# HengWeiBin/CenterFusionDetect3D

Hardware: AMD Instinct MI355X
Metric: frames/sec/GPU CenterFusion forward, 3x448x800 bs=16; 1/2/4/8-GPU scaling (higher is better)
Workload: dtype f32 storage + f32 accumulate; products as split-operand MFMA passes: f16x3 backbone/neck (3 passes), heads' first 3x3 layers fp16 main term + block-scaled FP6 e2m3 cross terms (1.5 passes), heads' 1x1 layers bf16x3; 1 GPU; Centerfusion_Middle (DLA-34 + DCNv2 neck + pc_dep frustum fusion, 7+4 heads) forward + NMS/top-100 decode + 2D->3D postProcess, bs=16/GPU, 3x448x800, 50-200 radar pts/frame, random-init weights; global_batch=16, parallelism=dp1 (batch shard, async all-gather of the final boxes)

## Files before the change

centerfusiondetect3d_amd/csrc/cf_heads.hip:

```cpp
#include <string>
#include "cf_common.h"
#include "cf_mx.h"

namespace {

typedef __bf16 bf16x8 __attribute__((ext_vector_type(8)));
typedef unsigned int u32x4 __attribute__((ext_vector_type(4)));
typedef unsigned int u32x2 __attribute__((ext_vector_type(2)));
typedef _Float16 hf16x8 __attribute__((ext_vector_type(8)));
typedef int i32x8 __attribute__((ext_vector_type(8)));

constexpr int HT_PX = 64;
constexpr int HT_C = 256;
constexpr int HT_ROWB = HT_C * 2 + 16;
constexpr int HT_PLANE = HT_PX * HT_ROWB;
constexpr int HT_LDS = 2 * HT_PLANE;

struct HeadTailK {
  const unsigned char* x;
  int x_stride;
  int M, HW;
  int n_heads;
  int n_hidden;
  const unsigned char* w_hidden[CF_MAX_HEADS][2];
// ... 36 lines not shown
        hi[e] = bf16_rne(v[e]);
      }
      unsigned char* o = xt + (ct * 16 + c16) * HT_ROWB + ch * 2;
      const u32x2 ph = {pack2(hi[0], hi[1]), pack2(hi[2], hi[3])};
      const u32x2 pl = {pack2(v[0] - hi[0], v[1] - hi[1]), pack2(v[2] - hi[2], v[3] - hi[3])};
      *reinterpret_cast<u32x2*>(o) = ph;
      *reinterpret_cast<u32x2*>(o + HT_PLANE) = pl;
    }
  }
}

struct TileMap {
  int b, y0, x0, H, W, sh = 4;
  __device__ __forceinline__ bool operator()(int px, int& bb, int& pix) const {
    const int y = y0 + (px >> sh), x = x0 + (px & ((1 << sh) - 1));
    if (y >= H || x >= W) return false;
    bb = b;
    pix = y * W + x;
    return true;
  }
};

constexpr int AT_SLOTS = CF_HEAD_AT_SLOTS;
__device__ __forceinline__ int at_slot_of(int ty, int tx) { return (ty % 3 == 0 && tx % 3 == 0) ? (ty / 3) * 6 + tx / 3 : -1; }
struct SlotMap {
  const int* slots;
  int M, HW, half;
  __device__ __forceinline__ bool operator()(int px, int& bb, int& pix) const {
    const int t = half * 64 + px, sl = at_slot_of(t >> 4, t & 15);
    if (sl < 0) return false;
    const int s = slots[sl];
    if ((unsigned)s >= (unsigned)M) return false;
    bb = s / HW;
    pix = s - bb * HW;
    return true;
  }
};

template <class PixMap, int CTS = 0xF>
__device__ __forceinline__ void head_tail_from_lds16(const HeadTailK& p, unsigned char* xt, int head, const PixMap& pm) {
  const int tid = threadIdx.x, lane = tid & 63, wave = tid >> 6;
  const int g = lane >> 4, c16 = lane & 15;
  for (int l = 0; l < p.n_hidden; ++l) {
    const unsigned char* w = p.w_hidden[head][l];
    const float* bias = p.b_hidden[head][l];
    f32x4 acc[4][4];
#pragma unroll
    for (int a = 0; a < 4; ++a)
#pragma unroll
      for (int b = 0; b < 4; ++b)
#pragma unroll
        for (int r = 0; r < 4; ++r) acc[a][b][r] = 0.0f;
    bf16x8 wh[2][4], wl[2][4];
#pragma unroll
    for (int rt = 0; rt < 4; ++rt) {
      wh[0][rt] = *wfrag(w, wave * 4 + rt, 0, 0, 8, lane);
      wl[0][rt] = *wfrag(w, wave * 4 + rt, 0, 1, 8, lane);
    }
#pragma unroll
    for (int ks = 0; ks < 8; ++ks) {
      if (ks + 1 < 8) {
#pragma unroll
        for (int rt = 0; rt < 4; ++rt) {
          wh[(ks + 1) & 1][rt] = *wfrag(w, wave * 4 + rt, ks + 1, 0, 8, lane);
          wl[(ks + 1) & 1][rt] = *wfrag(w, wave * 4 + rt, ks + 1, 1, 8, lane);
        }
      }
      bf16x8 xh[4], xl[4];
#pragma unroll
      for (int ct = 0; ct < 4; ++ct) {
        if (!((CTS >> ct) & 1)) continue;
        const unsigned char* row = xt + (ct * 16 + c16) * HT_ROWB + (ks * 32 + g * 8) * 2;
        xh[ct] = *reinterpret_cast<const bf16x8*>(row);
        xl[ct] = *reinterpret_cast<const bf16x8*>(row + HT_PLANE);
      }
#pragma unroll
      for (int rt = 0; rt < 4; ++rt)
#pragma unroll
        for (int ct = 0; ct < 4; ++ct)
          if ((CTS >> ct) & 1) acc[rt][ct] = __builtin_amdgcn_mfma_f32_16x16x32_bf16(wl[ks & 1][rt], xh[ct], acc[rt][ct], 0, 0, 0);
#pragma unroll
      for (int rt = 0; rt < 4; ++rt)
#pragma unroll
        for (int ct = 0; ct < 4; ++ct)
          if ((CTS >> ct) & 1) acc[rt][ct] = __builtin_amdgcn_mfma_f32_16x16x32_bf16(wh[ks & 1][rt], xl[ct], acc[rt][ct], 0, 0, 0);
#pragma unroll
      for (int rt = 0; rt < 4; ++rt)
#pragma unroll
        for (int ct = 0; ct < 4; ++ct)
          if ((CTS >> ct) & 1) acc[rt][ct] = __builtin_amdgcn_mfma_f32_16x16x32_bf16(wh[ks & 1][rt], xh[ct], acc[rt][ct], 0, 0, 0);
      __builtin_amdgcn_sched_barrier(0);
    }
    __syncthreads();
    store_hidden_tile16<false, CTS>(xt, acc, bias, wave, lane);
    __syncthreads();
  }

  f32x4 oacc[4];
#pragma unroll
  for (int b = 0; b < 4; ++b)
#pragma unroll
    for (int r = 0; r < 4; ++r) oacc[b][r] = 0.0f;
  {
    const unsigned char* w = p.w_out[head];
#pragma unroll
    for (int s2 = 0; s2 < 2; ++s2) {
      const int ks = wave * 2 + s2;
      const bf16x8 ah = *wfrag(w, 0, ks, 0, 8, lane), al = *wfrag(w, 0, ks, 1, 8, lane);
#pragma unroll
      for (int ct = 0; ct < 4; ++ct) {
        if (!((CTS >> ct) & 1)) continue;
        const unsigned char* row = xt + (ct * 16 + c16) * HT_ROWB + (ks * 32 + g * 8) * 2;
        const bf16x8 xh = *reinterpret_cast<const bf16x8*>(row);
// ... 25 lines not shown
      const float raw = red[n * HT_PX + px] + red[(16 + n) * HT_PX + px] + red[(32 + n) * HT_PX + px] +
                        red[(48 + n) * HT_PX + px] + bo[n];
      const size_t o = ((size_t)b * n_out + n) * p.HW + pix;
      float v = raw;
      if (act == CF_ACT_RELU) v = fmaxf(raw, 0.0f);
      else if (act == CF_ACT_SIGMOID_CLAMP) v = fminf(fmaxf(cf_sigmoid(raw), 1e-4f), 1.0f - 1e-4f);
      out[o] = v;
      if (act == CF_ACT_RAW_AND_SIGDEPTH) out2[o] = 1.0f / (cf_sigmoid(raw) + 1e-6f) - 1.0f;
    }
  }
}

constexpr int HP_ROWS = (8 + 2) * (16 + 2);
constexpr int HP_PX = 8 * 16;
constexpr int HP16_RED = 4 * 16 * HP_PX * 4;
constexpr int hp16_patch_bytes(bool pc) { return HP_ROWS * (4 * 64 + (pc ? 32 : 0) + 16); }
constexpr int HP_PCIMG_ROWB = 32 * 2 + 16;
constexpr int HP_PCIMG = HP_PX * 2 * HP_PCIMG_ROWB;
constexpr int hp16_pc_extra(bool pc) { return pc ? 16 + HP_PCIMG : 0; }
constexpr int hp16_lds(bool pc, bool hidden) {
  return hidden ? (HT_LDS > hp16_patch_bytes(pc) + hp16_pc_extra(pc) ? HT_LDS : hp16_patch_bytes(pc) + hp16_pc_extra(pc))
                : hp16_patch_bytes(pc) + hp16_pc_extra(pc) + HP16_RED;
}

struct HeadPatchK {
  HeadTailK t;
  const unsigned char* src[2];
  int src_c[2];
  int H, W, tiles_x, tiles_y, n_ks;
  int pc_skip;
  int hloop;
  const unsigned char* w_first[CF_MAX_HEADS];
  const float* b_first[CF_MAX_HEADS];
  const unsigned char* w_out_perm[CF_MAX_HEADS];
  float first_scale[CF_MAX_HEADS];
  const int* slot_pixels;
};

template <int NS, bool PC, bool TP, bool MX = false, int HID = -1, bool AT = false>
__global__ __launch_bounds__(256, 2) void head_patch16_kernel(HeadPatchK q) {
  static_assert(NS == 4, "64 feature channels");
  static_assert(!AT || !TP, "virtual tiles are laid out on the flat 8 x 16 tile");
  constexpr int MX_SLAB = 14592, PC_OFF = MX ? 272 : NS * 64;
  constexpr int TSH = TP ? 3 : 4, TMASK = (1 << TSH) - 1;
  constexpr int T_H = TP ? 16 : 8, T_W = TP ? 8 : 16, P_W = T_W + 2;
  static_assert((T_H + 2) * P_W == HP_ROWS, "both tile shapes have the same patch size");
  constexpr int ROWB = NS * 64 + (PC ? 32 : 0) + 16;
  constexpr int NKF = 9 * NS / 2;
  constexpr int NK = NKF + (PC ? 1 : 0);
  extern __shared__ __attribute__((aligned(16))) unsigned char xt[];
  const HeadTailK& p = q.t;
  const int tid = threadIdx.x, lane = tid & 63, wave = __builtin_amdgcn_readfirstlane(tid >> 6);
  const int g = lane >> 4;
  const int c16 = (MX && !TP) ? ((lane & 12) == 4 || (lane & 12) == 8 ? (((lane & 15) - 4) & 3) * 4 + (((lane & 15) - 4) >> 2)
                                                                      : (lane & 3) * 4 + 2 + ((lane & 15) >> 3))
                              : (lane & 15);
  const int per_img = q.tiles_x * q.tiles_y;
  const int per_head = AT ? per_img : per_img * (p.M / p.HW);
  const int hg = blockIdx.x / per_head;
  int rem = cf_xcd_remap(blockIdx.x - hg * per_head, per_head);
  const int head0 = hg * q.hloop, head1 = min(head0 + q.hloop, p.n_heads);
  const int b = rem / per_img;
  rem -= b * per_img;
  const int y0 = (rem / q.tiles_x) * T_H, x0 = (rem % q.tiles_x) * T_W;
  const int* const at_slots = AT ? q.slot_pixels + (size_t)rem * AT_SLOTS : nullptr;
  constexpr auto live = [](int ct) { return !AT || ct % 3 == 0; };
  auto at_src = [&](int row) -> int {
    const int pr = row / P_W, pc = row % P_W;
    if (pr >= 9) return -1;
    const int s = at_slots[(pr / 3) * 6 + pc / 3];
    if ((unsigned)s >= (unsigned)p.M) return -1;
    const int bb = s / p.HW, pix = s - bb * p.HW;
    const int y = pix / q.W + pr % 3 - 1, x = pix % q.W + pc % 3 - 1;
    if ((unsigned)y >= (unsigned)q.H || (unsigned)x >= (unsigned)q.W) return -1;
    return bb * p.HW + y * q.W + x;
  };
  if constexpr (AT) {
    int any = 0;
    for (int i = 0; i < AT_SLOTS; ++i) any |= (unsigned)at_slots[i] < (unsigned)p.M ? 1 : 0;
    if (!any) return;
  }

  if constexpr (MX) {
    constexpr int UPR = 17;
    constexpr int NIT = (HP_ROWS * UPR + 255) / 256;
    u32x4 v[NIT];
#pragma unroll
    for (int it = 0; it < NIT; ++it) {
      const int idx = tid + it * 256;
      const int row = idx / UPR, u = idx % UPR;
      const int y = y0 - 1 + row / P_W, x = x0 - 1 + row % P_W;
      v[it] = u32x4{0u, 0u, 0u, 0u};
      if constexpr (AT) {
        const int s = row < HP_ROWS ? at_src(row) : -1;
        if (s >= 0) v[it] = *reinterpret_cast<const u32x4*>(q.src[0] + (size_t)s * 272 + u * 16);
      } else
      if (row < HP_ROWS && (unsigned)y < (unsigned)q.H && (unsigned)x < (unsigned)q.W)
        v[it] = *reinterpret_cast<const u32x4*>(q.src[0] + (size_t)(b * p.HW + y * q.W + x) * 272 + u * 16);
    }
#pragma unroll
    for (int it = 0; it < NIT; ++it) {
      const int idx = tid + it * 256;
      const int row = idx / UPR, u = idx % UPR;
      if (row < HP_ROWS) *reinterpret_cast<u32x4*>(xt + row * ROWB + u * 16) = v[it];
    }
  } else {
    constexpr int UPR = NS * 4;
    constexpr int NIT = (HP_ROWS * UPR + 255) / 256;
    u32x4 v[NIT];
#pragma unroll
    for (int it = 0; it < NIT; ++it) {
      const int idx = tid + it * 256;
      const int row = idx / UPR, u = idx % UPR;
      const int y = y0 - 1 + row / P_W, x = x0 - 1 + row % P_W;
      v[it] = u32x4{0u, 0u, 0u, 0u};
      if constexpr (AT) {
        const int s = row < HP_ROWS ? at_src(row) : -1;
        if (s >= 0) v[it] = *reinterpret_cast<const u32x4*>(q.src[0] + ((size_t)s * 2 * q.src_c[0]) * 2 +
                                                             (u / (NS * 2)) * q.src_c[0] * 2 + (u % (NS * 2)) * 16);
      } else
      if (row < HP_ROWS && (unsigned)y < (unsigned)q.H && (unsigned)x < (unsigned)q.W)
        v[it] = *reinterpret_cast<const u32x4*>(q.src[0] + ((size_t)(b * p.HW + y * q.W + x) * 2 * q.src_c[0]) * 2 +
                                                (u / (NS * 2)) * q.src_c[0] * 2 + (u % (NS * 2)) * 16);
    }
#pragma unroll
    for (int it = 0; it < NIT; ++it) {
      const int idx = tid + it * 256;
      const int row = idx / UPR, u = idx % UPR;
      const int plane = u / (NS * 2), uu = u % (NS * 2);
      if (row < HP_ROWS) *reinterpret_cast<u32x4*>(xt + row * ROWB + (uu >> 1) * 64 + plane * 32 + (uu & 1) * 16) = v[it];
    }
  }
  unsigned* const pc_flags = reinterpret_cast<unsigned*>(xt + hp16_patch_bytes(PC));
  if (PC) {
    unsigned nz = 0u;
    for (int idx = tid; idx < HP_ROWS * 2; idx += 256) {
      const int row = idx >> 1, plane = idx & 1;
      const int y = y0 - 1 + row / P_W, x = x0 - 1 + row % P_W;
      u32x4 w = {0u, 0u, 0u, 0u};
      if constexpr (AT) {
        const int s = at_src(row);
        if (s >= 0) w = *reinterpret_cast<const u32x4*>(q.src[1] + ((size_t)s * 2 + plane) * q.src_c[1] * 2);
      } else
      if ((unsigned)y < (unsigned)q.H && (unsigned)x < (unsigned)q.W)
        w = *reinterpret_cast<const u32x4*>(q.src[1] + ((size_t)(b * p.HW + y * q.W + x) * 2 + plane) * q.src_c[1] * 2);
      *reinterpret_cast<u32x4*>(xt + row * ROWB + PC_OFF + plane * 16) = w;
      nz |= (w[0] | w[1] | w[2] | w[3]) & 0x7fff7fffu;
    }
    const bool wave_nz = __builtin_amdgcn_ballot_w64(nz != 0u) != 0ull;
    if (lane == 0) pc_flags[wave] = (wave_nz || !q.pc_skip) ? 1u : 0u;
  }

  int rowb[8];
#pragma unroll
  for (int ct = 0; ct < 8; ++ct)
    rowb[ct] = ((c16 >> TSH) * P_W + (c16 & TMASK)) * ROWB + ct * ((16 >> TSH) * P_W * ROWB);
  const int koff = (g >> 1) * 64 + (g & 1) * 16;
  unsigned char* const pcimg = xt + hp16_patch_bytes(PC) + 16;
  const int imgb = c16 * (2 * HP_PCIMG_ROWB) + g * 16;
  __syncthreads();
  bool pc_live = false;
  if (PC) {
    const u32x4 f = *reinterpret_cast<const u32x4*>(pc_flags);
    pc_live = __builtin_amdgcn_readfirstlane((int)(f[0] | f[1] | f[2] | f[3])) != 0;
  }
  if (PC && pc_live) {
    const int ipx = tid & (HP_PX - 1), plane = tid >> 7;
    const unsigned char* sp = xt + ((ipx >> TSH) * P_W + (ipx & TMASK)) * ROWB + PC_OFF + plane * 16;
    unsigned e[32];
#pragma unroll
    for (int t = 0; t < 9; ++t) {
      const u32x2 w = *reinterpret_cast<const u32x2*>(sp + ((t / 3) * P_W + t % 3) * ROWB);
      e[3 * t] = w[0] & 0xffffu;
      e[3 * t + 1] = w[0] >> 16;
      e[3 * t + 2] = w[1] & 0xffffu;
    }
#pragma unroll
    for (int k = 27; k < 32; ++k) e[k] = 0u;
    unsigned char* dp = pcimg + (ipx * 2 + plane) * HP_PCIMG_ROWB;
#pragma unroll
    for (int j = 0; j < 4; ++j)
      *reinterpret_cast<u32x4*>(dp + j * 16) = u32x4{e[8 * j] | (e[8 * j + 1] << 16), e[8 * j + 2] | (e[8 * j + 3] << 16),
                                                     e[8 * j + 4] | (e[8 * j + 5] << 16), e[8 * j + 6] | (e[8 * j + 7] << 16)};
    __syncthreads();
  }
  auto pc_kstep = [&](const bf16x8 (&ah)[4], const bf16x8 (&al)[4], f32x4 (&acc)[4][8]) __attribute__((always_inline)) {
#pragma unroll
    for (int hf = 0; hf < 2; ++hf) {
      bf16x8 xh[4], xl[4];
#pragma unroll
      for (int ct = 0; ct < 4; ++ct) {
        if (!live(4 * hf + ct)) continue;
        const unsigned char* r = pcimg + imgb + (4 * hf + ct) * (16 * 2 * HP_PCIMG_ROWB);
        xh[ct] = *reinterpret_cast<const bf16x8*>(r);
        xl[ct] = *reinterpret_cast<const bf16x8*>(r + HP_PCIMG_ROWB);
      }
#pragma unroll
      for (int rt = 0; rt < 4; ++rt)
#pragma unroll
        for (int ct = 0; ct < 4; ++ct)
          if (live(4 * hf + ct))
            acc[rt][4 * hf + ct] = __builtin_amdgcn_mfma_f32_16x16x32_bf16(al[rt], xh[ct], acc[rt][4 * hf + ct], 0, 0, 0);
#pragma unroll
      for (int rt = 0; rt < 4; ++rt)
#pragma unroll
        for (int ct = 0; ct < 4; ++ct)
// ... 160 lines not shown
        for (int ct = 0; ct < 4; ++ct)
          if (live(4 * hf + ct))
            acc[rt][4 * hf + ct] = __builtin_amdgcn_mfma_f32_16x16x32_bf16(wh[ks & 1][rt], xl[ct], acc[rt][4 * hf + ct], 0, 0, 0);
#pragma unroll
      for (int rt = 0; rt < 4; ++rt)
#pragma unroll
        for (int ct = 0; ct < 4; ++ct)
          if (live(4 * hf + ct))
            acc[rt][4 * hf + ct] = __builtin_amdgcn_mfma_f32_16x16x32_bf16(wh[ks & 1][rt], xh[ct], acc[rt][4 * hf + ct], 0, 0, 0);
    }
    __builtin_amdgcn_sched_barrier(0);
  }
  if (PC) {
    if (pc_live) pc_kstep(wh[NKF & 1], wl[NKF & 1], acc);
  }
  };

  if (HID < 0 ? p.n_hidden > 0 : HID == 1) {
    const int head = head0;
    f32x4 acc[4][8];
    first_layer(head, acc);
    __syncthreads();
#pragma unroll
    for (int half = 0; half < 2; ++half) {
      f32x4 a2[4][4];
#pragma unroll
      for (int rt = 0; rt < 4; ++rt)
#pragma unroll
        for (int ct = 0; ct < 4; ++ct) a2[rt][ct] = acc[rt][4 * half + ct];
      if constexpr (AT) {
        if (half == 0) store_hidden_tile16<MX, 0x9>(xt, a2, q.b_first[head], wave, lane, MX ? q.first_scale[head] : 1.0f, c16);
        else store_hidden_tile16<MX, 0x4>(xt, a2, q.b_first[head], wave, lane, MX ? q.first_scale[head] : 1.0f, c16);
      } else
      store_hidden_tile16<MX>(xt, a2, q.b_first[head], wave, lane, MX ? q.first_scale[head] : 1.0f, c16);
      if constexpr (MX) __builtin_amdgcn_sched_barrier(0);
      __syncthreads();
      if constexpr (AT) {
        if (half == 0) head_tail_from_lds16<SlotMap, 0x9>(p, xt, head, SlotMap{at_slots, p.M, p.HW, half});
        else head_tail_from_lds16<SlotMap, 0x4>(p, xt, head, SlotMap{at_slots, p.M, p.HW, half});
      }
      else head_tail_from_lds16(p, xt, head, TileMap{b, y0 + (64 >> TSH) * half, x0, q.H, q.W, TSH});
      __syncthreads();
    }
    return;
  }
  if constexpr (HID == 1) return;

  for (int head = head0; head < head1; ++head) {
  f32x4 acc[4][8];
  first_layer(head, acc);
  f32x4 oacc[8];
#pragma unroll
  for (int c = 0; c < 8; ++c)
#pragma unroll
    for (int r = 0; r < 4; ++r) oacc[c][r] = 0.0f;
  {
    const float* b1 = q.b_first[head] + wave * 64 + 4 * g;
    const unsigned char* wo = q.w_out_perm[head];
    const float fsc = MX ? q.first_scale[head] : 1.0f;
    (void)fsc;
#pragma unroll
    for (int s2 = 0; s2 < 2; ++s2) {
      const int ks2 = wave * 2 + s2;
      const bf16x8 ah = *wfrag(wo, 0, ks2, 0, 8, lane), al = *wfrag(wo, 0, ks2, 1, 8, lane);
      const f32x4 ba = *reinterpret_cast<const f32x4*>(b1 + 32 * s2);
      const f32x4 bb = *reinterpret_cast<const f32x4*>(b1 + 32 * s2 + 16);
#pragma unroll
      for (int ct = 0; ct < 8; ++ct) {
        if (!live(ct)) continue;
        float v[8], hi[8];
#pragma unroll
        for (int j = 0; j < 8; ++j) {
          const float bj = j < 4 ? ba[j] : bb[j - 4];
          v[j] = fmaxf(MX ? __builtin_fmaf(acc[2 * s2 + (j >> 2)][ct][j & 3], fsc, bj) : acc[2 * s2 + (j >> 2)][ct][j & 3] + bj, 0.0f);
          hi[j] = bf16_rne(v[j]);
        }
        const u32x4 ph = {pack2(hi[0], hi[1]), pack2(hi[2], hi[3]), pack2(hi[4], hi[5]), pack2(hi[6], hi[7])};
        const u32x4 pl = {pack2(v[0] - hi[0], v[1] - hi[1]), pack2(v[2] - hi[2], v[3] - hi[3]),
                          pack2(v[4] - hi[4], v[5] - hi[5]), pack2(v[6] - hi[6], v[7] - hi[7])};
        const bf16x8 xh = __builtin_bit_cast(bf16x8, ph), xl = __builtin_bit_cast(bf16x8, pl);
        oacc[ct] = __builtin_amdgcn_mfma_f32_16x16x32_bf16(al, xh, oacc[ct], 0, 0, 0);
        oacc[ct] = __builtin_amdgcn_mfma_f32_16x16x32_bf16(ah, xl, oacc[ct], 0, 0, 0);
        oacc[ct] = __builtin_amdgcn_mfma_f32_16x16x32_bf16(ah, xh, oacc[ct], 0, 0, 0);
      }
    }
  }
  const int n_out = p.n_out[head], act = p.act[head];
  float* red = reinterpret_cast<float*>(xt + hp16_patch_bytes(PC) + hp16_pc_extra(PC));
#pragma unroll
  for (int ct = 0; ct < 8; ++ct)
#pragma unroll
    for (int r = 0; r < 4; ++r) {
      const int n = 4 * g + r;
      if (live(ct) && n < n_out) red[(wave * 16 + n) * HP_PX + ct * 16 + c16] = oacc[ct][r];
    }
  __syncthreads();
  {
    const int px = tid & (HP_PX - 1);
    const int y = y0 + (px >> TSH), x = x0 + (px & TMASK);
    bool valid = y < q.H && x < q.W;
    int ob = b;
    size_t opix = (size_t)y * q.W + x;
    if constexpr (AT) {
      const int sl = at_slot_of(px >> 4, px & 15);
      const int s = sl >= 0 ? at_slots[sl] : -1;
      valid = (unsigned)s < (unsigned)p.M;
      ob = s / p.HW;
      opix = (size_t)(s - ob * p.HW);
    }
    if (valid) {
      const float* bo = p.b_out[head];
      float* out = p.out[head];
      float* out2 = p.out2[head];
      for (int n = tid >> 7; n < n_out; n += 2) {
        const float raw = red[n * HP_PX + px] + red[(16 + n) * HP_PX + px] + red[(32 + n) * HP_PX + px] +
                          red[(48 + n) * HP_PX + px] + bo[n];
        const size_t o = ((size_t)ob * n_out + n) * p.HW + opix;
        float v = raw;
        if (act == CF_ACT_RELU) v = fmaxf(raw, 0.0f);
        else if (act == CF_ACT_SIGMOID_CLAMP) v = fminf(fmaxf(cf_sigmoid(raw), 1e-4f), 1.0f - 1e-4f);
        out[o] = v;
        if (act == CF_ACT_RAW_AND_SIGDEPTH) out2[o] = 1.0f / (cf_sigmoid(raw) + 1e-6f) - 1.0f;
      }
    }
  }
  __syncthreads();
  }
}

__global__ __launch_bounds__(256) void pack_feat_mx_kernel(const float* __restrict__ x, int in_stride,
                                                           unsigned char* __restrict__ rows, long M, float scale) {
  const long t = (long)blockIdx.x * 256 + threadIdx.x;
  const long m = t >> 1;
  const int blk = (int)(t & 1);
  if (m >= M) return;
  const f32x4* src = reinterpret_cast<const f32x4*>(x + m * in_stride + 32 * blk);
  float v[32];
#pragma unroll
  for (int i = 0; i < 8; ++i) {
// ... 96 lines not shown
  CF_REQUIRE(mx || a->K_pad / 16 >= (a->n_src == 2 ? 38 : 36), "cf_head_fused: K_pad=%d too small for the 3x3 layout", a->K_pad);
  for (int i = 0; i < n_heads; ++i) {
    CF_REQUIRE(!mx || (a->first_scale[i] > 0.0f && a->first_scale[i] < 1e30f), "cf_head_fused: head %d: first_scale missing (mx)", i);
    hp.first_scale[i] = a->first_scale[i];
  }
  if (m16) {
    CF_REQUIRE(mx || (a->K_pad % 32 == 0 && a->K_pad / 32 >= (a->n_src == 2 ? 19 : 18)), "cf_head_fused: K_pad=%d (16x16x32 fragments)", a->K_pad);
    for (int i = 0; i < n_heads; ++i)
      CF_REQUIRE(a->tail.n_out[i] <= 16, "cf_head_fused: head %d: n_out=%d > 16 (the 16x16x32 kernels produce ONE 16-row output tile, with or without hidden layers)", i, a->tail.n_out[i]);
  }
  for (int i = 0; i < n_heads; ++i) {
    CF_REQUIRE(a->tail.n_hidden > 0 || a->w_out_perm[i], "cf_head_fused: head %d: w_out_perm missing", i);
    hp.w_out_perm[i] = reinterpret_cast<const unsigned char*>(a->w_out_perm[i]);
  }
  const long t_land = (long)((W + 15) / 16) * ((H + 7) / 8), t_port = (long)((W + 7) / 8) * ((H + 15) / 16);
  CF_REQUIRE(t_land * a->tail.B * n_heads < (1L << 31), "cf_head_fused: grid too large");
  CF_REQUIRE(m16, CF_HEAD_FORMS ": nothing reads 32x32x16 fragments (mfma16 = 0)");
  bool portrait = tile < 0 ? t_port < t_land : tile != 0;
  if (at) portrait = false;
  hp.pc_skip = pc_skip != 0;
  hp.tiles_x = portrait ? (W + 7) / 8 : (W + 15) / 16;
  hp.tiles_y = portrait ? (H + 15) / 16 : (H + 7) / 8;
  const int n_img = at ? 1 : a->tail.B;
  if (at) { hp.tiles_x = n_tiles; hp.tiles_y = 1; }
  int hloop = 1;
  if (a->tail.n_hidden == 0) {
    static const int slots = [] {
      int dev = 0, cus = 256;
      if (hipGetDevice(&dev) == hipSuccess) (void)hipDeviceGetAttribute(&cus, hipDeviceAttributeMultiprocessorCount, dev);
      return 2 * (cus > 0 ? cus : 256);
    }();
    const long tiles = (long)hp.tiles_x * hp.tiles_y * n_img;
    const int n = n_heads, cand[3] = {1, 2, (n + 1) / 2};
    double best = 0.0;
    for (int i = 0; i < 3; ++i) {
      const int h = cand[i] < 1 ? 1 : (cand[i] > n ? n : cand[i]);
      const double cost = (double)((tiles * ((n + h - 1) / h) + slots - 1) / slots) * (h + 0.25);
      if (i == 0 || cost < best - 1e-9) { best = cost; hloop = h; }
    }
  }
  hp.hloop = hloop;
  const long blocks = (long)hp.tiles_x * hp.tiles_y * n_img * ((n_heads + hloop - 1) / hloop);
  CF_REQUIRE(blocks < (1L << 31), "%s: grid too large", at ? "cf_head_fused_at" : "cf_head_fused");
  const bool hidden = a->tail.n_hidden > 0;
  const bool pc = a->n_src == 2;
  const int lds = hp16_lds(pc, hidden);
  auto launch = [&](auto kernel, CfLdsLimit& lim) {
    lim.ensure(kernel, lds, hp16_lds(pc, false));
    hipLaunchKernelGGL(kernel, dim3((unsigned)blocks), dim3(256), lds, (hipStream_t)stream, hp);
  };
  static CfLdsLimit lim16[4], limx[4], limxh[2], lim_at[4];
  if (at) {
    CF_REQUIRE(!mx || hidden == pc, "cf_head_fused_at: mx = 1 runs without hidden layers and pc_hm source, or with both (the forms "
                                    "the model's head groups take); pack other heads for bf16x3");
    if (mx && hidden) launch(head_patch16_kernel<4, true, false, true, 1, true>, lim_at[3]);
    else if (mx) launch(head_patch16_kernel<4, false, false, true, 0, true>, lim_at[2]);
    else if (pc) launch(head_patch16_kernel<4, true, false, false, -1, true>, lim_at[1]);
    else launch(head_patch16_kernel<4, false, false, false, -1, true>, lim_at[0]);
    return cf_check_launch("cf_head_fused_at");
  }
  if (mx && hidden) {
    CF_REQUIRE(pc, "cf_head_fused: mx = 1 with hidden layers needs the pc_hm source (n_src = 2); pack such heads for bf16x3");
    if (portrait) launch(head_patch16_kernel<4, true, true, true, 1>, limxh[1]);
    else launch(head_patch16_kernel<4, true, false, true, 1>, limxh[0]);
  } else if (mx) {
    if (pc && portrait) launch(head_patch16_kernel<4, true, true, true, 0>, limx[3]);
    else if (pc) launch(head_patch16_kernel<4, true, false, true, 0>, limx[2]);
    else if (portrait) launch(head_patch16_kernel<4, false, true, true, 0>, limx[1]);
    else launch(head_patch16_kernel<4, false, false, true, 0>, limx[0]);
  } else {
    if (pc && portrait) launch(head_patch16_kernel<4, true, true>, lim16[3]);
    else if (pc) launch(head_patch16_kernel<4, true, false>, lim16[2]);
    else if (portrait) launch(head_patch16_kernel<4, false, true>, lim16[1]);
    else launch(head_patch16_kernel<4, false, false>, lim16[0]);
  }
  return cf_check_launch("cf_head_fused");
}

// ... 54 lines not shown
```

centerfusiondetect3d_amd/plan.py:

```python
import ctypes as C
import weakref
from typing import Dict, List

import torch

from . import _lib, ops, packing
from .pending import PendingOutputs
from ._lib import (ACT_NONE, ACT_RELU, ACT_SIGMOID_CLAMP, ACT_RAW_AND_SIGDEPTH, LAYOUT_NHWC, LAYOUT_NCHW)
from .streams import _side_streams

SECONDARY_HEADS = ["velocity", "nuscenes_att", "depth2", "rotation2"]
AT_SLOTS = 18
AT_TIMED = ("at.topk", "at.peaks", "at.tables", "at.primary")


def feat_operand(model):
    if not model._heads_bf():
        return None
    return ((packing.MX_ROW,), torch.uint8) if model._mx_active else ((2, 64), torch.bfloat16)


def act_of(h):
    return ACT_SIGMOID_CLAMP if h == "heatmap" else (ACT_RAW_AND_SIGDEPTH if h in ("depth", "depth2") else ACT_NONE)

# ... 580 lines not shown
                    self.steps[self.frustum_step] = (lib.cf_frustum_assoc, self.tk_inds.data_ptr(), K, *geom)
            self._radar_outputs(y, out, heads, pc_dep, pc_hm)
        for name, (flops, px_flops, _) in self.group_flops.items():
            self.step_flops[name] = flops
        if at is None:
            self._launch(st)
        else:
            raw = tk[:3] if self.frustum else (None, None, None)
            fused = (hm.data_ptr(), B, heads["heatmap"], h4, w4, K, *raw, pk_s.data_ptr(), pk_i.data_ptr(), pk_c.data_ptr(),
                     at["tab_ab"].data_ptr() if self.frustum else None, at["tab_b"].data_ptr(), at["ws"].data_ptr())
            self._launch(st, self._at_seq(at, (_peaks_fused_and_checksum, lib, fused, peaks[3])))
            y = self._pending(y, model, written)
        if self.peaks_step is not None and peaks_on:
            hm._cf_peaks = (K, hm.data_ptr(), pk_s, pk_i, pk_c, pk_sum)
            if self._side is not None:
                for t in (hm, pk_s, pk_i, pk_c, pk_sum):
                    t.record_stream(self._side)
        return [y]

    def _at_seq(self, at, peaks):
        lib, idx = self.lib, self.step_index
        tab_b, n_b = at["tab_b"].data_ptr(), at["n_b"]
        tab_p, n_p = (at["tab_ab"].data_ptr(), at["n_ab"]) if self.frustum else (tab_b, n_b)
        HP_PX = 48
        extra = ([("at.topk", (_no_launch,), 0)] if self.frustum else []) + [
                  ("at.peaks", peaks, 0), ("at.tables", (_no_launch,), 0),
                  ("at.primary", (lib.cf_head_fused_at, C.byref(at["f_rest"]), tab_p, n_p), 0)]
        repl = {idx["tails.primary"]: (lib.cf_head_fused, C.byref(at["f_hm"]))}
        self.step_flops["tails.primary"] = at["flops_hm"]
        self.step_flops["at.primary"] = n_p * HP_PX * at["px_rest"]
        for name in ("tails.chained", "tails.secondary"):
            if name in idx:
                _, px_flops, f = self.group_flops[name]
                repl[idx[name]] = (lib.cf_head_fused_at, C.byref(f), tab_b, n_b)
                self.step_flops[name] = n_b * HP_PX * px_flops
        seq = []
        for i, (step, lane) in enumerate(zip(self.steps, self.lanes)):
            seq.append((i, repl.get(i, step), lane))
            if i == idx["tails.primary"]:
                seq += extra
        return seq

    def _pending(self, y, model, written):
        fwd = torch.cuda.current_stream(self.device)
        lib, dev = self.lib, self.device
        names = [n for n in ("tails.primary", "tails.chained", "tails.secondary") if n in self.step_index]
        blocks = []
        for n in names:
            f = self.group_flops[n][2]
            c = _lib.HeadFusedArgs()
            C.memmove(C.byref(c), C.byref(f), C.sizeof(f))
            blocks.append(c)
        bufs = {t.data_ptr(): t for n in names for t in self.group_srcs[n]}
        keep = [written, list(y.values()), self, model._packed, bufs]

        def materialise():
            with torch.cuda.device(dev):
                for c in blocks:
# ... 48 lines not shown
```

Baseline: 3180 frames/s.

## Pack listed AT pixels densely into 48-pixel workgroups with paired-head blocks

The attention-tail head kernels stop mapping listed pixels onto a sparse 8x16 virtual tile (one live pixel per 3x3 cell). They now pack 48 listed pixels contiguously per workgroup, each with its own 9-row neighbourhood patch. A small LDS table holds each pixel's flat index and packed y/x. The hidden chain deepens its weight prefetch to three k-steps, and a 512-thread paired-head variant runs two heads at once when the grid oversubscribes the CUs. This cuts wasted MFMA columns, gather work and block count for the sparse decode-time head evaluation, at the cost of more LDS per block, new occupancy heuristics and extra register pressure from the deeper prefetch.

```diff
diff --git a/centerfusiondetect3d_amd/csrc/cf_heads.hip b/centerfusiondetect3d_amd/csrc/cf_heads.hip
--- a/centerfusiondetect3d_amd/csrc/cf_heads.hip
+++ b/centerfusiondetect3d_amd/csrc/cf_heads.hip
@@ -82,22 +82,25 @@
 };
 
 constexpr int AT_SLOTS = CF_HEAD_AT_SLOTS;
-__device__ __forceinline__ int at_slot_of(int ty, int tx) { return (ty % 3 == 0 && tx % 3 == 0) ? (ty / 3) * 6 + tx / 3 : -1; }
+constexpr int AT_S = 48;
+constexpr int AT_CTS = (1 << (AT_S / 16)) - 1;
+constexpr int AT_AHEAD = 3;
+constexpr int AT_ROWS = 9 * AT_S;
+constexpr int AT_INFO = AT_S * 8;
 struct SlotMap {
-  const int* slots;
-  int M, HW, half;
+  const int* info;
+  int HW;
   __device__ __forceinline__ bool operator()(int px, int& bb, int& pix) const {
-    const int t = half * 64 + px, sl = at_slot_of(t >> 4, t & 15);
-    if (sl < 0) return false;
-    const int s = slots[sl];
-    if ((unsigned)s >= (unsigned)M) return false;
+    if (px >= AT_S) return false;
+    const int s = info[2 * px];
+    if (s < 0) return false;
     bb = s / HW;
     pix = s - bb * HW;
     return true;
   }
 };
 
-template <class PixMap, int CTS = 0xF>
+template <class PixMap, int CTS = 0xF, int AHEAD = 1>
 __device__ __forceinline__ void head_tail_from_lds16(const HeadTailK& p, unsigned char* xt, int head, const PixMap& pm) {
   const int tid = threadIdx.x, lane = tid & 63, wave = tid >> 6;
   const int g = lane >> 4, c16 = lane & 15;
@@ -111,19 +114,22 @@
       for (int b = 0; b < 4; ++b)
 #pragma unroll
         for (int r = 0; r < 4; ++r) acc[a][b][r] = 0.0f;
-    bf16x8 wh[2][4], wl[2][4];
-#pragma unroll
-    for (int rt = 0; rt < 4; ++rt) {
-      wh[0][rt] = *wfrag(w, wave * 4 + rt, 0, 0, 8, lane);
-      wl[0][rt] = *wfrag(w, wave * 4 + rt, 0, 1, 8, lane);
-    }
+    constexpr int NB = AHEAD + 1;
+    bf16x8 wh[NB][4], wl[NB][4];
+#pragma unroll
+    for (int a = 0; a < AHEAD; ++a)
+#pragma unroll
+      for (int rt = 0; rt < 4; ++rt) {
+        wh[a][rt] = *wfrag(w, wave * 4 + rt, a, 0, 8, lane);
+        wl[a][rt] = *wfrag(w, wave * 4 + rt, a, 1, 8, lane);
+      }
 #pragma unroll
     for (int ks = 0; ks < 8; ++ks) {
-      if (ks + 1 < 8) {
+      if (ks + AHEAD < 8) {
 #pragma unroll
         for (int rt = 0; rt < 4; ++rt) {
-          wh[(ks + 1) & 1][rt] = *wfrag(w, wave * 4 + rt, ks + 1, 0, 8, lane);
-          wl[(ks + 1) & 1][rt] = *wfrag(w, wave * 4 + rt, ks + 1, 1, 8, lane);
+          wh[(ks + AHEAD) % NB][rt] = *wfrag(w, wave * 4 + rt, ks + AHEAD, 0, 8, lane);
+          wl[(ks + AHEAD) % NB][rt] = *wfrag(w, wave * 4 + rt, ks + AHEAD, 1, 8, lane);
         }
       }
       bf16x8 xh[4], xl[4];
@@ -138,17 +144,17 @@
       for (int rt = 0; rt < 4; ++rt)
 #pragma unroll
         for (int ct = 0; ct < 4; ++ct)
-          if ((CTS >> ct) & 1) acc[rt][ct] = __builtin_amdgcn_mfma_f32_16x16x32_bf16(wl[ks & 1][rt], xh[ct], acc[rt][ct], 0, 0, 0);
+          if ((CTS >> ct) & 1) acc[rt][ct] = __builtin_amdgcn_mfma_f32_16x16x32_bf16(wl[ks % NB][rt], xh[ct], acc[rt][ct], 0, 0, 0);
 #pragma unroll
       for (int rt = 0; rt < 4; ++rt)
 #pragma unroll
         for (int ct = 0; ct < 4; ++ct)
-          if ((CTS >> ct) & 1) acc[rt][ct] = __builtin_amdgcn_mfma_f32_16x16x32_bf16(wh[ks & 1][rt], xl[ct], acc[rt][ct], 0, 0, 0);
+          if ((CTS >> ct) & 1) acc[rt][ct] = __builtin_amdgcn_mfma_f32_16x16x32_bf16(wh[ks % NB][rt], xl[ct], acc[rt][ct], 0, 0, 0);
 #pragma unroll
       for (int rt = 0; rt < 4; ++rt)
 #pragma unroll
         for (int ct = 0; ct < 4; ++ct)
-          if ((CTS >> ct) & 1) acc[rt][ct] = __builtin_amdgcn_mfma_f32_16x16x32_bf16(wh[ks & 1][rt], xh[ct], acc[rt][ct], 0, 0, 0);
+          if ((CTS >> ct) & 1) acc[rt][ct] = __builtin_amdgcn_mfma_f32_16x16x32_bf16(wh[ks % NB][rt], xh[ct], acc[rt][ct], 0, 0, 0);
       __builtin_amdgcn_sched_barrier(0);
     }
     __syncthreads();
@@ -220,6 +226,16 @@
   return hidden ? (HT_LDS > hp16_patch_bytes(pc) + hp16_pc_extra(pc) ? HT_LDS : hp16_patch_bytes(pc) + hp16_pc_extra(pc))
                 : hp16_patch_bytes(pc) + hp16_pc_extra(pc) + HP16_RED;
 }
+constexpr int at_patch_bytes(bool pc) { return AT_ROWS * (4 * 64 + (pc ? 32 : 0) + 16); }
+constexpr int at_pc_extra(bool pc) { return pc ? 16 + AT_S * 2 * HP_PCIMG_ROWB : 0; }
+constexpr int AT_RED = 4 * 16 * AT_S * 4;
+constexpr int at_lds(bool pc, bool hidden, bool pair = false) {
+  return at_patch_bytes(pc) + at_pc_extra(pc) + AT_INFO + (hidden ? 0 : (pair ? 2 : 1) * AT_RED);
+}
+constexpr int CU_LDS = 160 * 1024;
+static_assert(at_lds(true, false) <= CU_LDS && at_lds(true, true) <= CU_LDS && at_lds(false, false, true) <= CU_LDS,
+              "an AT workgroup's patch, operand image and partial sums fit one CU's LDS");
+static_assert(at_patch_bytes(false) >= HT_LDS, "the hidden chain's tile lies inside the AT patch");
 
 struct HeadPatchK {
   HeadTailK t;
@@ -233,22 +249,30 @@
   const unsigned char* w_out_perm[CF_MAX_HEADS];
   float first_scale[CF_MAX_HEADS];
   const int* slot_pixels;
+  int n_slots;
 };
 
-template <int NS, bool PC, bool TP, bool MX = false, int HID = -1, bool AT = false>
-__global__ __launch_bounds__(256, 2) void head_patch16_kernel(HeadPatchK q) {
+template <int NS, bool PC, bool TP, bool MX = false, int HID = -1, bool AT = false, bool PAIR = false>
+__global__ __launch_bounds__(PAIR ? 512 : 256, PAIR ? 1 : 2) void head_patch16_kernel(HeadPatchK q) {
+  static_assert(!PAIR || (AT && MX && !PC && HID == 0), "paired heads: the mx listed-pixel form without hidden layers");
+  constexpr int NT = PAIR ? 512 : 256;
   static_assert(NS == 4, "64 feature channels");
-  static_assert(!AT || !TP, "virtual tiles are laid out on the flat 8 x 16 tile");
+  static_assert(!AT || !TP, "listed pixels have no tile orientation");
   constexpr int MX_SLAB = 14592, PC_OFF = MX ? 272 : NS * 64;
   constexpr int TSH = TP ? 3 : 4, TMASK = (1 << TSH) - 1;
-  constexpr int T_H = TP ? 16 : 8, T_W = TP ? 8 : 16, P_W = T_W + 2;
-  static_assert((T_H + 2) * P_W == HP_ROWS, "both tile shapes have the same patch size");
+  constexpr int T_H = TP ? 16 : 8, T_W = TP ? 8 : 16, P_W = AT ? 3 : T_W + 2;
+  static_assert(AT || (T_H + 2) * P_W == HP_ROWS, "both tile shapes have the same patch size");
   constexpr int ROWB = NS * 64 + (PC ? 32 : 0) + 16;
+  constexpr int NROWS = AT ? AT_ROWS : HP_ROWS, NPX = AT ? AT_S : HP_PX;
+  constexpr int PATCH = NROWS * ROWB, INFO_OFF = PATCH + (PC ? 16 + NPX * 2 * HP_PCIMG_ROWB : 0), RED_OFF = INFO_OFF + (AT ? AT_INFO : 0);
+  static_assert(AT ? PATCH == at_patch_bytes(PC) && INFO_OFF == PATCH + at_pc_extra(PC)
+                   : PATCH == hp16_patch_bytes(PC) && RED_OFF == PATCH + hp16_pc_extra(PC), "the launcher's LDS figures");
   constexpr int NKF = 9 * NS / 2;
   constexpr int NK = NKF + (PC ? 1 : 0);
   extern __shared__ __attribute__((aligned(16))) unsigned char xt[];
   const HeadTailK& p = q.t;
-  const int tid = threadIdx.x, lane = tid & 63, wave = __builtin_amdgcn_readfirstlane(tid >> 6);
+  const int tid = threadIdx.x, lane = tid & 63, wave = PAIR ? __builtin_amdgcn_readfirstlane(tid >> 6) & 3 : __builtin_amdgcn_readfirstlane(tid >> 6);
+  const int grp = PAIR ? __builtin_amdgcn_readfirstlane(tid >> 8) : 0;
   const int g = lane >> 4;
   const int c16 = (MX && !TP) ? ((lane & 12) == 4 || (lane & 12) == 8 ? (((lane & 15) - 4) & 3) * 4 + (((lane & 15) - 4) >> 2)
                                                                       : (lane & 3) * 4 + 2 + ((lane & 15) >> 3))
@@ -261,25 +285,62 @@
   const int b = rem / per_img;
   rem -= b * per_img;
   const int y0 = (rem / q.tiles_x) * T_H, x0 = (rem % q.tiles_x) * T_W;
-  const int* const at_slots = AT ? q.slot_pixels + (size_t)rem * AT_SLOTS : nullptr;
-  constexpr auto live = [](int ct) { return !AT || ct % 3 == 0; };
+  const int at_first = AT ? rem * AT_S : 0;
+  int* const at_info = reinterpret_cast<int*>(xt + INFO_OFF);
+  constexpr auto live = [](int ct) { return !AT || ct < AT_S / 16; };
   auto at_src = [&](int row) -> int {
-    const int pr = row / P_W, pc = row % P_W;
-    if (pr >= 9) return -1;
-    const int s = at_slots[(pr / 3) * 6 + pc / 3];
-    if ((unsigned)s >= (unsigned)p.M) return -1;
-    const int bb = s / p.HW, pix = s - bb * p.HW;
-    const int y = pix / q.W + pr % 3 - 1, x = pix % q.W + pc % 3 - 1;
-    if ((unsigned)y >= (unsigned)q.H || (unsigned)x >= (unsigned)q.W) return -1;
-    return bb * p.HW + y * q.W + x;
+    const int sl = row / 9, t = row - sl * 9;
+    const u32x2 inf = *reinterpret_cast<const u32x2*>(at_info + 2 * sl);
+    const int dy = t / 3 - 1, dx = t % 3 - 1;
+    const int y = (int)(inf[1] >> 16) + dy, x = (int)(inf[1] & 0xffffu) + dx;
+    if ((int)inf[0] < 0 || (unsigned)y >= (unsigned)q.H || (unsigned)x >= (unsigned)q.W) return -1;
+    return (int)inf[0] + dy * q.W + dx;
   };
   if constexpr (AT) {
-    int any = 0;
-    for (int i = 0; i < AT_SLOTS; ++i) any |= (unsigned)at_slots[i] < (unsigned)p.M ? 1 : 0;
-    if (!any) return;
-  }
-
-  if constexpr (MX) {
+    if (tid < AT_S) {
+      const int s = at_first + tid < q.n_slots ? q.slot_pixels[at_first + tid] : -1;
+      int flat = -1, yx = 0;
+      if ((unsigned)s < (unsigned)p.M) {
+        const int pix = s % p.HW, y = pix / q.W;
+        flat = s;
+        yx = (y << 16) | (pix - y * q.W);
+      }
+      at_info[2 * tid] = flat;
+      at_info[2 * tid + 1] = yx;
+    }
+    __syncthreads();
+    static_assert(AT_S <= 64, "one lane per entry");
+    if (__builtin_amdgcn_ballot_w64(lane < AT_S && at_info[2 * (lane < AT_S ? lane : 0)] >= 0) == 0ull) return;
+  }
+
+  if constexpr (AT) {
+    constexpr int UPR = MX ? 17 : NS * 4;
+    constexpr int NU = AT_ROWS * UPR, NIT = (NU + NT - 1) / NT, BATCH = 8;
+#pragma unroll
+    for (int b0 = 0; b0 < NIT; b0 += BATCH) {
+      u32x4 v[BATCH];
+#pragma unroll
+      for (int j = 0; j < BATCH; ++j) {
+        if (b0 + j >= NIT) continue;
+        const int idx = min(tid + (b0 + j) * NT, NU - 1);
+        const int row = idx / UPR, u = idx % UPR;
+        const int s = at_src(row), sc = max(s, 0);
+        v[j] = MX ? *reinterpret_cast<const u32x4*>(q.src[0] + (size_t)sc * 272 + u * 16)
+                  : *reinterpret_cast<const u32x4*>(q.src[0] + ((size_t)sc * 2 * q.src_c[0]) * 2 +
+                                                    (u / (NS * 2)) * q.src_c[0] * 2 + (u % (NS * 2)) * 16);
+        if (s < 0) v[j] = u32x4{0u, 0u, 0u, 0u};
+      }
+#pragma unroll
+      for (int j = 0; j < BATCH; ++j) {
+        const int idx = tid + (b0 + j) * NT;
+        const int row = idx / UPR, u = idx % UPR;
+        const int plane = u / (NS * 2), uu = u % (NS * 2);
+        if (b0 + j < NIT && idx < NU)
+          *reinterpret_cast<u32x4*>(xt + row * ROWB + (MX ? u * 16 : (uu >> 1) * 64 + plane * 32 + (uu & 1) * 16)) = v[j];
+      }
+      __builtin_amdgcn_sched_barrier(0);
+    }
+  } else if constexpr (MX) {
     constexpr int UPR = 17;
     constexpr int NIT = (HP_ROWS * UPR + 255) / 256;
     u32x4 v[NIT];
@@ -289,10 +350,6 @@
       const int row = idx / UPR, u = idx % UPR;
       const int y = y0 - 1 + row / P_W, x = x0 - 1 + row % P_W;
       v[it] = u32x4{0u, 0u, 0u, 0u};
-      if constexpr (AT) {
-        const int s = row < HP_ROWS ? at_src(row) : -1;
-        if (s >= 0) v[it] = *reinterpret_cast<const u32x4*>(q.src[0] + (size_t)s * 272 + u * 16);
-      } else
       if (row < HP_ROWS && (unsigned)y < (unsigned)q.H && (unsigned)x < (unsigned)q.W)
         v[it] = *reinterpret_cast<const u32x4*>(q.src[0] + (size_t)(b * p.HW + y * q.W + x) * 272 + u * 16);
     }
@@ -312,11 +369,6 @@
       const int row = idx / UPR, u = idx % UPR;
       const int y = y0 - 1 + row / P_W, x = x0 - 1 + row % P_W;
       v[it] = u32x4{0u, 0u, 0u, 0u};
-      if constexpr (AT) {
-        const int s = row < HP_ROWS ? at_src(row) : -1;
-        if (s >= 0) v[it] = *reinterpret_cast<const u32x4*>(q.src[0] + ((size_t)s * 2 * q.src_c[0]) * 2 +
-                                                             (u / (NS * 2)) * q.src_c[0] * 2 + (u % (NS * 2)) * 16);
-      } else
       if (row < HP_ROWS && (unsigned)y < (unsigned)q.H && (unsigned)x < (unsigned)q.W)
         v[it] = *reinterpret_cast<const u32x4*>(q.src[0] + ((size_t)(b * p.HW + y * q.W + x) * 2 * q.src_c[0]) * 2 +
                                                 (u / (NS * 2)) * q.src_c[0] * 2 + (u % (NS * 2)) * 16);
@@ -329,17 +381,30 @@
       if (row < HP_ROWS) *reinterpret_cast<u32x4*>(xt + row * ROWB + (uu >> 1) * 64 + plane * 32 + (uu & 1) * 16) = v[it];
     }
   }
-  unsigned* const pc_flags = reinterpret_cast<unsigned*>(xt + hp16_patch_bytes(PC));
+  unsigned* const pc_flags = reinterpret_cast<unsigned*>(xt + PATCH);
   if (PC) {
     unsigned nz = 0u;
-    for (int idx = tid; idx < HP_ROWS * 2; idx += 256) {
+    if constexpr (AT) {
+      constexpr int NITP = (NROWS * 2 + 255) / 256;
+      u32x4 w[NITP];
+#pragma unroll
+      for (int it = 0; it < NITP; ++it) {
+        const int idx = min(tid + it * 256, NROWS * 2 - 1);
+        const int s = at_src(idx >> 1);
+        w[it] = *reinterpret_cast<const u32x4*>(q.src[1] + ((size_t)max(s, 0) * 2 + (idx & 1)) * q.src_c[1] * 2);
+        if (s < 0 || tid + it * 256 >= NROWS * 2) w[it] = u32x4{0u, 0u, 0u, 0u};
+      }
+#pragma unroll
+      for (int it = 0; it < NITP; ++it) {
+        const int idx = tid + it * 256;
+        if (idx < NROWS * 2) *reinterpret_cast<u32x4*>(xt + (idx >> 1) * ROWB + PC_OFF + (idx & 1) * 16) = w[it];
+        nz |= (w[it][0] | w[it][1] | w[it][2] | w[it][3]) & 0x7fff7fffu;
+      }
+    } else
+    for (int idx = tid; idx < NROWS * 2; idx += 256) {
       const int row = idx >> 1, plane = idx & 1;
       const int y = y0 - 1 + row / P_W, x = x0 - 1 + row % P_W;
       u32x4 w = {0u, 0u, 0u, 0u};
-      if constexpr (AT) {
-        const int s = at_src(row);
-        if (s >= 0) w = *reinterpret_cast<const u32x4*>(q.src[1] + ((size_t)s * 2 + plane) * q.src_c[1] * 2);
-      } else
       if ((unsigned)y < (unsigned)q.H && (unsigned)x < (unsigned)q.W)
         w = *reinterpret_cast<const u32x4*>(q.src[1] + ((size_t)(b * p.HW + y * q.W + x) * 2 + plane) * q.src_c[1] * 2);
       *reinterpret_cast<u32x4*>(xt + row * ROWB + PC_OFF + plane * 16) = w;
@@ -352,9 +417,9 @@
   int rowb[8];
 #pragma unroll
   for (int ct = 0; ct < 8; ++ct)
-    rowb[ct] = ((c16 >> TSH) * P_W + (c16 & TMASK)) * ROWB + ct * ((16 >> TSH) * P_W * ROWB);
+    rowb[ct] = AT ? (ct * 16 + c16) * (9 * ROWB) : ((c16 >> TSH) * P_W + (c16 & TMASK)) * ROWB + ct * ((16 >> TSH) * P_W * ROWB);
   const int koff = (g >> 1) * 64 + (g & 1) * 16;
-  unsigned char* const pcimg = xt + hp16_patch_bytes(PC) + 16;
+  unsigned char* const pcimg = xt + PATCH + 16;
   const int imgb = c16 * (2 * HP_PCIMG_ROWB) + g * 16;
   __syncthreads();
   bool pc_live = false;
@@ -363,8 +428,9 @@
     pc_live = __builtin_amdgcn_readfirstlane((int)(f[0] | f[1] | f[2] | f[3])) != 0;
   }
   if (PC && pc_live) {
-    const int ipx = tid & (HP_PX - 1), plane = tid >> 7;
-    const unsigned char* sp = xt + ((ipx >> TSH) * P_W + (ipx & TMASK)) * ROWB + PC_OFF + plane * 16;
+    const int ipx = AT ? tid % AT_S : tid & (HP_PX - 1), plane = AT ? tid / AT_S : tid >> 7;
+    const unsigned char* sp = xt + (AT ? ipx * 9 : (ipx >> TSH) * P_W + (ipx & TMASK)) * ROWB + PC_OFF + plane * 16;
+    if (!AT || plane < 2) {
     unsigned e[32];
 #pragma unroll
     for (int t = 0; t < 9; ++t) {
@@ -380,6 +446,7 @@
     for (int j = 0; j < 4; ++j)
       *reinterpret_cast<u32x4*>(dp + j * 16) = u32x4{e[8 * j] | (e[8 * j + 1] << 16), e[8 * j + 2] | (e[8 * j + 3] << 16),
                                                      e[8 * j + 4] | (e[8 * j + 5] << 16), e[8 * j + 6] | (e[8 * j + 7] << 16)};
+    }
     __syncthreads();
   }
   auto pc_kstep = [&](const bf16x8 (&ah)[4], const bf16x8 (&al)[4], f32x4 (&acc)[4][8]) __attribute__((always_inline)) {
@@ -586,23 +653,18 @@
     first_layer(head, acc);
     __syncthreads();
 #pragma unroll
-    for (int half = 0; half < 2; ++half) {
+    for (int half = 0; half < (AT ? 1 : 2); ++half) {
       f32x4 a2[4][4];
 #pragma unroll
       for (int rt = 0; rt < 4; ++rt)
 #pragma unroll
         for (int ct = 0; ct < 4; ++ct) a2[rt][ct] = acc[rt][4 * half + ct];
-      if constexpr (AT) {
-        if (half == 0) store_hidden_tile16<MX, 0x9>(xt, a2, q.b_first[head], wave, lane, MX ? q.first_scale[head] : 1.0f, c16);
-        else store_hidden_tile16<MX, 0x4>(xt, a2, q.b_first[head], wave, lane, MX ? q.first_scale[head] : 1.0f, c16);
-      } else
+      if constexpr (AT) store_hidden_tile16<MX, AT_CTS>(xt, a2, q.b_first[head], wave, lane, MX ? q.first_scale[head] : 1.0f, c16);
+      else
       store_hidden_tile16<MX>(xt, a2, q.b_first[head], wave, lane, MX ? q.first_scale[head] : 1.0f, c16);
       if constexpr (MX) __builtin_amdgcn_sched_barrier(0);
       __syncthreads();
-      if constexpr (AT) {
-        if (half == 0) head_tail_from_lds16<SlotMap, 0x9>(p, xt, head, SlotMap{at_slots, p.M, p.HW, half});
-        else head_tail_from_lds16<SlotMap, 0x4>(p, xt, head, SlotMap{at_slots, p.M, p.HW, half});
-      }
+      if constexpr (AT) head_tail_from_lds16<SlotMap, AT_CTS, AT_AHEAD>(p, xt, head, SlotMap{at_info, p.HW});
       else head_tail_from_lds16(p, xt, head, TileMap{b, y0 + (64 >> TSH) * half, x0, q.H, q.W, TSH});
       __syncthreads();
     }
@@ -610,7 +672,8 @@
   }
   if constexpr (HID == 1) return;
 
-  for (int head = head0; head < head1; ++head) {
+  for (int hd = head0; hd < head1; hd += PAIR ? 2 : 1) {
+  const int head = PAIR ? min(hd + grp, head1 - 1) : hd;
   f32x4 acc[4][8];
   first_layer(head, acc);
   f32x4 oacc[8];
@@ -650,25 +713,24 @@
     }
   }
   const int n_out = p.n_out[head], act = p.act[head];
-  float* red = reinterpret_cast<float*>(xt + hp16_patch_bytes(PC) + hp16_pc_extra(PC));
+  float* red = reinterpret_cast<float*>(xt + RED_OFF + (PAIR ? grp * AT_RED : 0));
 #pragma unroll
   for (int ct = 0; ct < 8; ++ct)
 #pragma unroll
     for (int r = 0; r < 4; ++r) {
       const int n = 4 * g + r;
-      if (live(ct) && n < n_out) red[(wave * 16 + n) * HP_PX + ct * 16 + c16] = oacc[ct][r];
+      if (live(ct) && n < n_out) red[(wave * 16 + n) * NPX + ct * 16 + c16] = oacc[ct][r];
     }
   __syncthreads();
   {
-    const int px = tid & (HP_PX - 1);
+    const int px = AT ? tid & 63 : tid & (HP_PX - 1);
     const int y = y0 + (px >> TSH), x = x0 + (px & TMASK);
     bool valid = y < q.H && x < q.W;
     int ob = b;
     size_t opix = (size_t)y * q.W + x;
     if constexpr (AT) {
-      const int sl = at_slot_of(px >> 4, px & 15);
-      const int s = sl >= 0 ? at_slots[sl] : -1;
-      valid = (unsigned)s < (unsigned)p.M;
+      const int s = px < AT_S ? at_info[2 * px] : -1;
+      valid = s >= 0;
       ob = s / p.HW;
       opix = (size_t)(s - ob * p.HW);
     }
@@ -676,9 +738,9 @@
       const float* bo = p.b_out[head];
       float* out = p.out[head];
       float* out2 = p.out2[head];
-      for (int n = tid >> 7; n < n_out; n += 2) {
-        const float raw = red[n * HP_PX + px] + red[(16 + n) * HP_PX + px] + red[(32 + n) * HP_PX + px] +
-                          red[(48 + n) * HP_PX + px] + bo[n];
+      for (int n = AT ? wave : tid >> 7; n < n_out; n += AT ? 4 : 2) {
+        const float raw = red[n * NPX + px] + red[(16 + n) * NPX + px] + red[(32 + n) * NPX + px] +
+                          red[(48 + n) * NPX + px] + bo[n];
         const size_t o = ((size_t)ob * n_out + n) * p.HW + opix;
         float v = raw;
         if (act == CF_ACT_RELU) v = fmaxf(raw, 0.0f);
@@ -821,38 +883,48 @@
   hp.tiles_x = portrait ? (W + 7) / 8 : (W + 15) / 16;
   hp.tiles_y = portrait ? (H + 15) / 16 : (H + 7) / 8;
   const int n_img = at ? 1 : a->tail.B;
-  if (at) { hp.tiles_x = n_tiles; hp.tiles_y = 1; }
+  const bool hidden = a->tail.n_hidden > 0;
+  const bool pc = a->n_src == 2;
+  if (at) {
+    CF_REQUIRE((long)n_tiles * AT_SLOTS < (1L << 31), "cf_head_fused_at: n_tiles=%d too large", n_tiles);
+    CF_REQUIRE(H < 32768 && W < 65536, "cf_head_fused_at: map %d x %d too large (an entry's row and column share one word)", H, W);
+    hp.n_slots = n_tiles * AT_SLOTS;
+    hp.tiles_x = (hp.n_slots + AT_S - 1) / AT_S;
+    hp.tiles_y = 1;
+  }
+  static const int cus = [] {
+    int dev = 0, n = 256;
+    if (hipGetDevice(&dev) == hipSuccess) (void)hipDeviceGetAttribute(&n, hipDeviceAttributeMultiprocessorCount, dev);
+    return n > 0 ? n : 256;
+  }();
+  const bool pair = at && mx && !pc && !hidden && n_heads > 1 && (long)hp.tiles_x * n_heads > cus;
+  const int lds = at ? at_lds(pc, hidden, pair) : hp16_lds(pc, hidden);
   int hloop = 1;
   if (a->tail.n_hidden == 0) {
-    static const int slots = [] {
-      int dev = 0, cus = 256;
-      if (hipGetDevice(&dev) == hipSuccess) (void)hipDeviceGetAttribute(&cus, hipDeviceAttributeMultiprocessorCount, dev);
-      return 2 * (cus > 0 ? cus : 256);
-    }();
+    const int per_cu = at ? (CU_LDS / lds > 1 ? CU_LDS / lds : 1) : 2;
+    const int slots = per_cu * cus;
     const long tiles = (long)hp.tiles_x * hp.tiles_y * n_img;
-    const int n = n_heads, cand[3] = {1, 2, (n + 1) / 2};
+    const int n = n_heads, cand[3] = {pair ? 2 : 1, 2, (n + 1) / 2};
     double best = 0.0;
     for (int i = 0; i < 3; ++i) {
       const int h = cand[i] < 1 ? 1 : (cand[i] > n ? n : cand[i]);
-      const double cost = (double)((tiles * ((n + h - 1) / h) + slots - 1) / slots) * (h + 0.25);
+      const double cost = (double)((tiles * ((n + h - 1) / h) + slots - 1) / slots) * ((pair ? (h + 1) / 2 : h) + 0.25);
       if (i == 0 || cost < best - 1e-9) { best = cost; hloop = h; }
     }
   }
   hp.hloop = hloop;
   const long blocks = (long)hp.tiles_x * hp.tiles_y * n_img * ((n_heads + hloop - 1) / hloop);
   CF_REQUIRE(blocks < (1L << 31), "%s: grid too large", at ? "cf_head_fused_at" : "cf_head_fused");
-  const bool hidden = a->tail.n_hidden > 0;
-  const bool pc = a->n_src == 2;
-  const int lds = hp16_lds(pc, hidden);
   auto launch = [&](auto kernel, CfLdsLimit& lim) {
-    lim.ensure(kernel, lds, hp16_lds(pc, false));
-    hipLaunchKernelGGL(kernel, dim3((unsigned)blocks), dim3(256), lds, (hipStream_t)stream, hp);
+    lim.ensure(kernel, lds, at ? at_lds(pc, false, pair) : hp16_lds(pc, false));
+    hipLaunchKernelGGL(kernel, dim3((unsigned)blocks), dim3(pair ? 512 : 256), lds, (hipStream_t)stream, hp);
   };
-  static CfLdsLimit lim16[4], limx[4], limxh[2], lim_at[4];
+  static CfLdsLimit lim16[4], limx[4], limxh[2], lim_at[5];
   if (at) {
     CF_REQUIRE(!mx || hidden == pc, "cf_head_fused_at: mx = 1 runs without hidden layers and pc_hm source, or with both (the forms "
                                     "the model's head groups take); pack other heads for bf16x3");
     if (mx && hidden) launch(head_patch16_kernel<4, true, false, true, 1, true>, lim_at[3]);
+    else if (mx && pair) launch(head_patch16_kernel<4, false, false, true, 0, true, true>, lim_at[4]);
     else if (mx) launch(head_patch16_kernel<4, false, false, true, 0, true>, lim_at[2]);
     else if (pc) launch(head_patch16_kernel<4, true, false, false, -1, true>, lim_at[1]);
     else launch(head_patch16_kernel<4, false, false, false, -1, true>, lim_at[0]);
diff --git a/centerfusiondetect3d_amd/plan.py b/centerfusiondetect3d_amd/plan.py
--- a/centerfusiondetect3d_amd/plan.py
+++ b/centerfusiondetect3d_amd/plan.py
@@ -626,18 +626,21 @@
         lib, idx = self.lib, self.step_index
         tab_b, n_b = at["tab_b"].data_ptr(), at["n_b"]
         tab_p, n_p = (at["tab_ab"].data_ptr(), at["n_ab"]) if self.frustum else (tab_b, n_b)
-        HP_PX = 48
+        AT_S = 48
+
+        def cols(n_tiles):
+            return -(-n_tiles * AT_SLOTS // AT_S) * AT_S
         extra = ([("at.topk", (_no_launch,), 0)] if self.frustum else []) + [
                   ("at.peaks", peaks, 0), ("at.tables", (_no_launch,), 0),
                   ("at.primary", (lib.cf_head_fused_at, C.byref(at["f_rest"]), tab_p, n_p), 0)]
         repl = {idx["tails.primary"]: (lib.cf_head_fused, C.byref(at["f_hm"]))}
         self.step_flops["tails.primary"] = at["flops_hm"]
-        self.step_flops["at.primary"] = n_p * HP_PX * at["px_rest"]
+        self.step_flops["at.primary"] = cols(n_p) * at["px_rest"]
         for name in ("tails.chained", "tails.secondary"):
             if name in idx:
                 _, px_flops, f = self.group_flops[name]
                 repl[idx[name]] = (lib.cf_head_fused_at, C.byref(f), tab_b, n_b)
-                self.step_flops[name] = n_b * HP_PX * px_flops
+                self.step_flops[name] = cols(n_b) * px_flops
         seq = []
         for i, (step, lane) in enumerate(zip(self.steps, self.lanes)):
             seq.append((i, repl.get(i, step), lane))
```

Measured after the change: 3200 frames/s, median of 6. About the same (+0.6%).
